# Division/CUDA-RayTracing

Measured on AMD Instinct MI355X. Metric: Mrays/s + achieved HBM GB/s, Stanford bunny 1920x1080x8spp @1/2/4/8 GPU, higher is better.
Workload: dtype f32

## Files before the change

### cuda-raytracing_amd/__init__.py

```python
import contextlib
import ctypes
import os

import numpy as np
import torch

PKG_DIR = os.path.dirname(os.path.abspath(__file__))
ROOT_DIR = os.path.dirname(PKG_DIR)
LIB_PATH = os.path.join(PKG_DIR, "librt_hip.so")
EXP_LIB_PATH = os.path.join(PKG_DIR, "librt_hip_exp.so")
ASSETS_DIR = os.path.join(ROOT_DIR, "assets")

RT_RENDER_STATS = 1
RT_RENDER_VALIDATE = 16
TRACERS = {"fast": 0, "ref": 2, "flat": 4, "wavefront": 8}
STAT_NAMES = ("segments", "nodes", "tri_tests", "tri_accepts", "sphere_accepts", "hits", "misses", "cycles_tree_cut",
              "wave_small_iters", "lane_small", "wave_big_tris", "lane_big_tris", "wave_segment_iters",
              "lane_segments", "tree_nodes", "tree_tri_tests", "cycles_small", "cycles_big", "cycles_total",
              "rounds_coop", "rounds_shared", "coop_rays", "cycles_tree_clusters", "cycles_tree_tris",
              "big_tests", "twin_decided", "twin_tests", "wave_big_iters", "defer_end2", "defer_redo", None, None)
STAT_COUNT = len(STAT_NAMES)
SCENES = {"bunny": 0, "bunny4": 1, "plane1m": 2}

REFERENCE_SPP = 5
# ... 248 lines not shown
    "rt_scene_camera": (None, [_P, ctypes.POINTER(GPUCamera)]),
    "rt_scene_host_arrays": (_SZ, [_P, ctypes.POINTER(_P), ctypes.POINTER(_SZ), ctypes.POINTER(_P),
                                   ctypes.POINTER(_SZ), ctypes.POINTER(_P), ctypes.POINTER(_SZ), ctypes.POINTER(_P)]),
    "rt_scene_bvh_max_depth": (_I, [_P]),
    "rt_scene_materials": (_I, [_P, _P, ctypes.POINTER(_SZ)]),
    "rt_scene_spheres": (_I, [_P, _P, ctypes.POINTER(_SZ)]),
    "rt_bvh_build_device": (_I, [_P, _U32, _P, _U32, _P, _P, ctypes.POINTER(_U32), ctypes.POINTER(_I), _P]),
    "rt_scene_mirror_info": (_I, [_P, ctypes.POINTER(_SZ), ctypes.POINTER(_SZ), ctypes.POINTER(_SZ)]),
    "rt_scene_mirror_copy": (_I, [_P, _P, _P, _P]),
    "rt_scene_mirror_nodes": (_I, [_P, _P, ctypes.POINTER(_SZ)]),
    "rt_scene_mirror_face_leaf": (_I, [_P, _P, ctypes.POINTER(_SZ)]),
    "rt_scene_mirror_twins": (_I, [_P, _P, ctypes.POINTER(_SZ), _P, ctypes.POINTER(_SZ)]),
    "rt_mirror_build_check": (_I, [_P, _SZ, _P, _SZ, _P, _SZ, _P, _SZ, _P, ctypes.POINTER(ctypes.c_int)]),
    "rt_cluster_cull_host": (_I, [_P, _P, ctypes.c_float, _P]),
    "rt_twin_check_host": (_I, [_P, _P, _P]),
    "rt_variant_host": (None, [_P, _P]),
    "rt_family_has_mode_host": (_I, [_I, _I]),
    "rt_xorwow_jump_matrix": (_I, [_I, ctypes.POINTER(ctypes.c_uint32)]),
    "rt_xorwow_init_host": (None, [_U32, _U64, _P]),
}

_lib = None


class RTError(RuntimeError):
    pass


def lib():
    global _lib
# ... 148 lines not shown
        _check(lib().rt_scene_mirror_face_leaf(self.handle, None, ctypes.byref(n)), "rt_scene_mirror_face_leaf")
        out = np.zeros(n.value, dtype=np.uint32)
        if n.value:
            _check(lib().rt_scene_mirror_face_leaf(self.handle, out.ctypes.data, ctypes.byref(n)), "rt_scene_mirror_face_leaf")
        return out

    def mirror_twins(self):
        import numpy as np
        nq, nu = ctypes.c_size_t(), ctypes.c_size_t()
        _check(lib().rt_scene_mirror_twins(self.handle, None, ctypes.byref(nq), None, ctypes.byref(nu)), "rt_scene_mirror_twins")
        q = np.zeros((nq.value, 28), dtype=np.float32)
        u = np.zeros((nu.value, 16), dtype=np.float32)
        _check(lib().rt_scene_mirror_twins(self.handle, q.ctypes.data, ctypes.byref(nq), u.ctypes.data, ctypes.byref(nu)),
               "rt_scene_mirror_twins")
        return q, u

    def materials(self):
        n = ctypes.c_size_t()
        _check(lib().rt_scene_materials(self.handle, None, ctypes.byref(n)), "rt_scene_materials")
        out = np.zeros((n.value, 16), dtype=np.float32)
        if n.value:
            _check(lib().rt_scene_materials(self.handle, out.ctypes.data, ctypes.byref(n)), "rt_scene_materials")
        return out

    def spheres(self):
        n = ctypes.c_size_t()
        _check(lib().rt_scene_spheres(self.handle, None, ctypes.byref(n)), "rt_scene_spheres")
        out = np.zeros((n.value, 8), dtype=np.float32)
        if n.value:
            _check(lib().rt_scene_spheres(self.handle, out.ctypes.data, ctypes.byref(n)), "rt_scene_spheres")
# ... 1033 lines not shown
```

### cuda-raytracing_amd/csrc/host_hooks.hip

```cpp
#include <hip/hip_runtime.h>

#include "rt_abi.h"
#include "rt_device.h"
#include "rt_math.h"
#include "rt_common.h"
#include "leaftree.h"
#include "rt_fast.h"
#include "mirror.h"
#include "rt_render.h"

static_assert(MIRROR_BIG_LEAF == (uint32_t)rtfast::BIG, "pair records exist for exactly the big leaves");

extern "C" int rt_experimental_loaded() { return rtk::experimental_kernels() ? 1 : 0; }

extern "C" int rt_twin_check_host(const float rec[12], const float o[3], const float nd[3]) {
    using rtm::f3;
    const f3 O = rtm::mk(o[0], o[1], o[2]), N = rtm::mk(nd[0], nd[1], nd[2]), v0 = rtm::mk(rec[0], rec[1], rec[2]);
    const f3 e1 = rtm::mk(rec[3], rec[4], rec[5]), e2 = rtm::mk(rec[6], rec[7], rec[8]);
    auto glm = [&](f3 a, f3 b, float* det, float* u, float* v, float* uv) {
        const f3 p = rtm::cross(N, b);
        *det = rtm::dot(a, p);
        const f3 dist = rtm::sub(O, v0);
        *u = rtm::dot(dist, p);
        *v = rtm::dot(N, rtm::cross(dist, a));
        *uv = *u + *v;
    };
    auto ok = [](float det, float u, float v, float uv) {
        const bool neg = signbit(det);
        const float ad = fabsf(det), su = neg ? -u : u, sv = neg ? -v : v, suv = neg ? -uv : uv;
        return ad > 1.1920928955078125e-07f && !(su < 0.0f || su > ad) && !(sv < 0.0f || suv > ad);
    };
    float d, u, v, uv, d2, u2, v2, uv2;
    glm(e1, e2, &d, &u, &v, &uv);
    glm(e2, e1, &d2, &u2, &v2, &uv2);
    const f3 dist = rtm::sub(O, v0);
    const float dn = (fabsf(dist.x) + fabsf(dist.y)) + fabsf(dist.z);
    float kd, ke;
    rt_twin_bounds(rec, &kd, &ke);
    return (rtfast::twin_rejected(d, u, v, uv, dn, kd, ke) ? 1 : 0) | (ok(d2, u2, v2, uv2) ? 2 : 0) | (ok(d, u, v, uv) ? 4 : 0);
}

extern "C" void rt_variant_host(const int32_t in[9], int32_t out[5]) {
    const rtk::VariantInput vi{(uint32_t)in[0], in[1] != 0, in[2] != 0, in[3] != 0, in[4] != 0,
                               in[5] != 0, in[6] != 0, in[7], in[8] != 0};
    const rtk::Variant v = rtk::choose_variant(vi);
    out[0] = v.family, out[1] = v.mode, out[2] = v.stack, out[3] = v.needs_plugin, out[4] = v.use_entry;
}

template <int... MODES>
static bool one_of(int mode) { return ((mode == MODES) || ...); }
extern "C" int rt_family_has_mode_host(int family, int mode) {
    switch (family) {
#define RT_FAMILY_CASE(FAM, NAME, STATS, ...) case rtk::FAM: return one_of<__VA_ARGS__>(mode);
        RT_FAST_FAMILIES(RT_FAMILY_CASE)
// ... 19 lines not shown
```

### cuda-raytracing_amd/csrc/mirror.cpp

```cpp
#include "mirror.h"

#include <cstdlib>
#include <functional>

#include "leaftree.h"

#include <algorithm>
#include <atomic>
#include <cmath>
#include <cstring>
#include <map>
#include <mutex>
#include <stdexcept>
#include <string>

namespace {
void put_flat(float* o, const float* p0, const float* p1, const float* p2, uint32_t face) {
    o[0] = p0[0], o[1] = p0[1], o[2] = p0[2];
    o[3] = p1[0] - p0[0], o[4] = p1[1] - p0[1], o[5] = p1[2] - p0[2];
    o[6] = p2[0] - p0[0], o[7] = p2[1] - p0[1], o[8] = p2[2] - p0[2];
    std::memcpy(&o[9], &face, 4);
    o[10] = o[11] = 0.0f;
}
void put_pair(float* q, const float* a, const float* b) {
// ... 4 lines not shown
    std::memcpy(&q[19], &b[9], 4);
}
}

void rt_twin_bounds(const float* r, float* kd, float* ke) {
    const double U = std::ldexp(1.0, -24);
    const double n1 = std::fabs((double)r[3]) + std::fabs((double)r[4]) + std::fabs((double)r[5]);
    const double n2 = std::fabs((double)r[6]) + std::fabs((double)r[7]) + std::fabs((double)r[8]);
    const double w = 1.0 + std::ldexp(1.0, -20);
    *kd = (float)(10.0001 * U * n1 * n2 * w * w);
    *ke = (float)(10.0001 * U * std::max(n1, n2) * w * w);
}

namespace {
bool build_twins(const float* tris, uint32_t first, uint32_t count, std::vector<float>& quads,
                 std::vector<float>& units, uint32_t* nq, uint32_t* nu) {
    if (count >= 0xffffu) return false;
    auto key = [&](uint32_t i, bool swapped) {
        const float* r = &tris[(size_t)(first + i) * 12];
        std::string k(reinterpret_cast<const char*>(r), 12);
        k.append(reinterpret_cast<const char*>(r + (swapped ? 6 : 3)), 12);
        k.append(reinterpret_cast<const char*>(r + (swapped ? 3 : 6)), 12);
        return k;
    };
    std::map<std::string, std::vector<uint32_t>> by;
    for (uint32_t i = 0; i < count; i++) by[key(i, false)].push_back(i);
    std::vector<char> used(count, 0);
    std::vector<std::pair<uint32_t, uint32_t>> un;
    for (uint32_t i = 0; i < count; i++) {
        if (used[i]) continue;
        used[i] = 1;
// ... 31 lines not shown
        float kd, ke;
        rt_twin_bounds(ra, &kd, &ke);
        q[20] = un[u].second == none ? -1.0f : kd, q[22] = ke;
        rt_twin_bounds(rb, &kd, &ke);
        q[21] = (!hb || un[u + 1].second == none) ? -1.0f : kd, q[23] = ke;
        const uint32_t wa = packed(un[u].first, un[u].second), wb = hb ? packed(un[u + 1].first, un[u + 1].second) : none;
        const uint32_t fa = face(un[u].second), fb = hb ? face(un[u + 1].second) : none;
        std::memcpy(&q[24], &wa, 4);
        std::memcpy(&q[25], &wb, 4);
        std::memcpy(&q[26], &fa, 4);
        std::memcpy(&q[27], &fb, 4);
        quads.insert(quads.end(), q, q + 28);
    }
    *nq = (uint32_t)((un.size() + 1) / 2);
    *nu = (uint32_t)un.size();
    return true;
}
}

void rt_build_mirror(const GPUBVHNode* nodes, size_t node_count, const uint32_t* fi, size_t index_count,
                     const GPUFace* faces, size_t face_count, const GPUVertex* verts, size_t vertex_count,
                     MirrorHost* out) {
    auto bad = [](const char* what) { throw std::runtime_error(std::string("mirror: ") + what); };
    out->tris.assign(index_count * 12, 0.0f);
    for (size_t i = 0; i < index_count; i++) {
        const uint32_t f = fi[i];
        if (f >= face_count) bad("face index out of range");
        const GPUFace& fc = faces[f];
        if (fc.v0 >= vertex_count || fc.v1 >= vertex_count || fc.v2 >= vertex_count) bad("vertex index out of range");
        put_flat(&out->tris[i * 12], verts[fc.v0].position, verts[fc.v1].position, verts[fc.v2].position, f);
// ... 68 lines not shown
        rt_get_build_options(&opt);
        if (nd.prim_count >= opt.leaf_tree_min) {
            LeafTreeParams prm;
            prm.cut_clusters = opt.cut_clusters;
            prm.split_angle = opt.split_angle;
            prm.cluster_max = opt.cluster_max;
            po = rt_build_leaf_tree(&out->tris[(size_t)nd.first_index * 12], nd.prim_count, prm, out->tree, out->ltris);
            rt_build_leaf_flat(out->tree, po, prm, out->flat);
            if (out->ltris.size() / 12 >= (1u << 26)) bad("leaf trees too large (record index >= 2^26)");
            roots.push_back(po);
            pf = 2;
            std::memcpy(&lead[10], &po, 4);
            std::memcpy(&lead[11], &pf, 4);
            continue;
        }
        float scr[20];
        rt_build_options so;
        rt_get_build_options(&so);
        LeafTreeParams sp;
        sp.split_angle = so.split_angle;
        pf = 1;
        if (so.leaf_screens && rt_build_leaf_screen(&out->tris[(size_t)nd.first_index * 12], nd.prim_count, sp, scr)) {
            out->pairs.insert(out->pairs.end(), scr, scr + 20);
            pf = 3;
            out->screens++;
        }
        po = (uint32_t)(out->pairs.size() / 20);
        std::memcpy(&lead[10], &po, 4);
        std::memcpy(&lead[11], &pf, 4);
        for (uint32_t j = 0; j < nd.prim_count; j += 2) {
            float q[20];
            put_pair(q, &out->tris[((size_t)nd.first_index + j) * 12],
                     j + 1 < nd.prim_count ? &out->tris[((size_t)nd.first_index + j + 1) * 12] : nullptr);
            out->pairs.insert(out->pairs.end(), q, q + 20);
        }
        const uint32_t qb = (uint32_t)(out->quads.size() / 28), ub = (uint32_t)(out->units.size() / 16);
        uint32_t nq = 0, nu = 0;
        if (twins_ok && build_twins(out->tris.data(), nd.first_index, nd.prim_count, out->quads, out->units, &nq, &nu)) {
            float* second = &out->tris[((size_t)nd.first_index + 1) * 12];
            float* third = &out->tris[((size_t)nd.first_index + 2) * 12];
            std::memcpy(&second[10], &qb, 4);
            std::memcpy(&second[11], &nq, 4);
            std::memcpy(&third[10], &ub, 4);
            std::memcpy(&third[11], &nu, 4);
        }
    }
    const uint32_t nl = (uint32_t)(out->ltris.size() / 12);
    for (uint32_t r : roots) std::memcpy(&out->tree[(size_t)r * 16 + 12], &nl, 4);
    rt_build_treelets(nodes, node_count, out->treelets);
    rt_build_private_nodes(nodes, node_count, out->nodes);
    out->face_leaf.clear();
    if (!out->pairs.empty() || !out->tree.empty()) {
        std::vector<uint32_t> fl(face_count, FACE_NO_LEAF);
        const size_t nn = out->nodes.size() / 8;
        for (size_t k = 0; k < nn; k++) {
            uint32_t first, count;
            std::memcpy(&first, &out->nodes[k * 8 + 6], 4);
            std::memcpy(&count, &out->nodes[k * 8 + 7], 4);
            if (count == 0 || (size_t)first + count > index_count) continue;
// ... 244 lines not shown
```

### cuda-raytracing_amd/csrc/rt_fast.h

```cpp
#pragma once

#include "rt_variant.h"

namespace rtfast {

constexpr int BIG = 8;
constexpr int WAVE = 64;

using rtm::f3;

struct Ray {
    f3 o, d, nd, r;
    bool fast;
};

__device__ __forceinline__ bool in_range_or_zero(float v, float lo, float hi) {
    const float a = fabsf(v);
    return v == 0.0f || (a >= lo && a <= hi);
}

__device__ __forceinline__ Ray make_ray(f3 o, f3 d, f3 nd, bool scene_fast) {
    Ray R;
    R.o = o, R.d = d, R.nd = nd;
    R.r = rtm::mk(1.0f / d.x, 1.0f / d.y, 1.0f / d.z);
// ... 200 lines not shown
            return true;
        }
    }
    return false;
}

__device__ __forceinline__ bool tri_ok(float det, float u, float v, float uv) {
    const float eps = 1.1920928955078125e-07f;
    const uint32_t sgn = __float_as_uint(det) & 0x80000000u;
    const float adet = fabsf(det);
    const float su = __uint_as_float(__float_as_uint(u) ^ sgn);
    const float sv = __uint_as_float(__float_as_uint(v) ^ sgn);
    const float suv = __uint_as_float(__float_as_uint(uv) ^ sgn);
    return adet > eps && !(su < 0.0f || su > adet) && !(sv < 0.0f || suv > adet);
}

__device__ __forceinline__ bool tri_accept(f3 o, f3 nd, float4 A, float4 B, float4 Cc, float best, float* t_o,
                                           float* bx, float* by, bool* nan) {
    const f3 e1 = rtm::mk(A.w, B.x, B.y), e2 = rtm::mk(B.z, B.w, Cc.x);
    const f3 p = rtm::cross(nd, e2);
    const float det = rtm::dot(e1, p);
    const f3 dist = rtm::sub(o, rtm::mk(A.x, A.y, A.z));
    const float u = rtm::dot(dist, p);
    const f3 perp = rtm::cross(dist, e1);
    const float v = rtm::dot(nd, perp);
    const float uv = u + v;
    if (!tri_ok(det, u, v, uv)) return false;
    const float inv_det = 1.0f / det;
    const float t = rtm::dot(e2, perp) * inv_det;
    *nan = *nan || (t != t);
// ... 21 lines not shown
}
__device__ __forceinline__ Pair ld_pair_scalar(ConstF4 base, uint32_t p) {
    return make_pair(base[5 * p], base[5 * p + 1], base[5 * p + 2], base[5 * p + 3], base[5 * p + 4]);
}
__device__ __forceinline__ Pair ld_pair(const float4* base, uint32_t p) {
#if defined(RT_ADDR64)
    const f4v* q = reinterpret_cast<const f4v*>(base) + 5 * (size_t)p;
#else
    const f4v* q = reinterpret_cast<const f4v*>(reinterpret_cast<const char*>(base) + p * 80u);
#endif
    return make_pair(q[0], q[1], q[2], q[3], q[4]);
}

struct PairEval {
    f2 det, u, v, uv, qx, qy, qz;
    f2 dn;
};
__device__ __forceinline__ PairEval pair_eval(f3 o, f3 nd, const Pair& P) {
    const f2 ndx = nd.x, ndy = nd.y, ndz = nd.z;
    const f2 px = ndy * P.e2z - P.e2y * ndz;
    const f2 py = ndz * P.e2x - P.e2z * ndx;
    const f2 pz = ndx * P.e2y - P.e2x * ndy;
    PairEval E;
    E.det = (P.e1x * px + P.e1y * py) + P.e1z * pz;
    const f2 dx = o.x - P.v0x, dy = o.y - P.v0y, dz = o.z - P.v0z;
    E.u = (dx * px + dy * py) + dz * pz;
    E.qx = dy * P.e1z - P.e1y * dz;
    E.qy = dz * P.e1x - P.e1z * dx;
    E.qz = dx * P.e1y - P.e1x * dy;
    E.v = (ndx * E.qx + ndy * E.qy) + ndz * E.qz;
    E.uv = E.u + E.v;
    E.dn = f2{(fabsf(dx.x) + fabsf(dy.x)) + fabsf(dz.x), (fabsf(dx.y) + fabsf(dy.y)) + fabsf(dz.y)};
    return E;
}

__device__ __forceinline__ float pair_t(const Pair& P, const PairEval& E, int k, float* inv) {
    const float det = k ? E.det.y : E.det.x;
    *inv = 1.0f / det;
    const f3 e2 = k ? rtm::mk(P.e2x.y, P.e2y.y, P.e2z.y) : rtm::mk(P.e2x.x, P.e2y.x, P.e2z.x);
    const f3 q = k ? rtm::mk(E.qx.y, E.qy.y, E.qz.y) : rtm::mk(E.qx.x, E.qy.x, E.qz.x);
    return rtm::dot(e2, q) * *inv;
}

__device__ __forceinline__ void pair_test(const Ray& R, const Pair& P, Hit& h) {
    const PairEval E = pair_eval(R.o, R.nd, P);
    const bool oka = tri_ok(E.det.x, E.u.x, E.v.x, E.uv.x);
    const bool okb = tri_ok(E.det.y, E.u.y, E.v.y, E.uv.y);
// ... 1 lines not shown
        float inv;
        const float t = pair_t(P, E, 0, &inv);
        if (!(t >= h.best || t < 0.0f)) h.best = t, h.kind = 2, h.id = P.fa, h.bx = E.u.x * inv, h.by = E.v.x * inv;
    }
    if (okb) {
        float inv;
        const float t = pair_t(P, E, 1, &inv);
        if (!(t >= h.best || t < 0.0f)) h.best = t, h.kind = 2, h.id = P.fb, h.bx = E.u.y * inv, h.by = E.v.y * inv;
    }
}

extern "C" __device__ uint32_t __ockl_wfred_min_u32(uint32_t);

constexpr uint32_t NO_POS = 0xffffffffu;

RT_HD bool twin_rejected(float det, float u, float v, float uv, float dn, float kd, float ke) {
    const bool neg = signbit(det);
    const float ad = fabsf(det);
    const float su = neg ? -u : u, sv = neg ? -v : v, suv = neg ? -uv : uv;
    if (!(ad + fabsf(su) + fabsf(sv) + dn < 0x1p100f)) return false;
    const float m = ke * dn + 0x1p-90f;
    const float kdd = kd + 0x1p-90f;
    const float top = (ad + kdd) * (1.0f + 0x1p-20f);
    if (top <= 1.1920928955078125e-07f) return true;
    if (!(ad > kdd * (1.0f + 0x1p-20f))) return false;
    if (sv < -m || su < -m) return true;
    if (sv > (ad + kdd + m) * (1.0f + 0x1p-20f)) return true;
    return suv * (1.0f - 0x1p-20f) > (ad + kdd + 2.001f * m) * (1.0f + 0x1p-20f);
}

__device__ __forceinline__ void offer(float t, uint32_t pos, uint32_t id, float bx, float by, Hit& h, uint32_t& bpos,
                                      bool& nan) {
    if (t != t) {
        nan = true;
        return;
    }
    const bool take = (t >= 0.0f) & ((t < h.best) | ((t == h.best) & (bpos != NO_POS) & (pos < bpos)));
    if (take) h.best = t, h.kind = 2, h.id = id, h.bx = bx, h.by = by, bpos = pos;
}

__device__ __forceinline__ void tri_offer(f3 o, f3 nd, f3 v0, f3 e1, f3 e2, uint32_t pos, uint32_t face, Hit& h,
                                          uint32_t& bpos, bool& nan) {
    const f3 p = rtm::cross(nd, e2);
    const float det = rtm::dot(e1, p);
    const f3 dist = rtm::sub(o, v0);
    const float u = rtm::dot(dist, p);
    const f3 perp = rtm::cross(dist, e1);
    const float v = rtm::dot(nd, perp);
    if (tri_ok(det, u, v, u + v)) {
        const float inv_det = 1.0f / det;
        offer(rtm::dot(e2, perp) * inv_det, pos, face, u * inv_det, v * inv_det, h, bpos, nan);
    }
}

template <bool TIMING, class C>
__device__ __forceinline__ void quad_test(f3 o, f3 nd, const Pair& P, f4v bnd, ConstF4 q6, Hit& h, uint32_t& bpos,
                                          bool& nan, C& c) {
    const PairEval E = pair_eval(o, nd, P);
    const bool oka = tri_ok(E.det.x, E.u.x, E.v.x, E.uv.x), okb = tri_ok(E.det.y, E.u.y, E.v.y, E.uv.y);
    const bool twa = bnd.x >= 0.0f && !twin_rejected(E.det.x, E.u.x, E.v.x, E.uv.x, E.dn.x, bnd.x, bnd.z);
    const bool twb = bnd.y >= 0.0f && !twin_rejected(E.det.y, E.u.y, E.v.y, E.uv.y, E.dn.y, bnd.y, bnd.w);
    if (TIMING) {
        c.big_tests += 2;
        c.tw_test += (uint32_t)twa + (uint32_t)twb;
        c.tw_dec += (uint32_t)(bnd.x >= 0.0f && !twa) + (uint32_t)(bnd.y >= 0.0f && !twb);
    }
    if (oka || okb || twa || twb) {
        const f4v W = *q6;
        const uint32_t wa = __float_as_uint(W.x), wb = __float_as_uint(W.y);
        if (oka) {
            float inv;
            const float t = pair_t(P, E, 0, &inv);
            offer(t, wa & 0xffffu, P.fa, E.u.x * inv, E.v.x * inv, h, bpos, nan);
        }
        if (okb) {
            float inv;
            const float t = pair_t(P, E, 1, &inv);
            offer(t, wb & 0xffffu, P.fb, E.u.y * inv, E.v.y * inv, h, bpos, nan);
        }
        if (twa)
            tri_offer(o, nd, rtm::mk(P.v0x.x, P.v0y.x, P.v0z.x), rtm::mk(P.e2x.x, P.e2y.x, P.e2z.x),
                      rtm::mk(P.e1x.x, P.e1y.x, P.e1z.x), wa >> 16, __float_as_uint(W.z), h, bpos, nan);
        if (twb)
            tri_offer(o, nd, rtm::mk(P.v0x.y, P.v0y.y, P.v0z.y), rtm::mk(P.e2x.y, P.e2y.y, P.e2z.y),
                      rtm::mk(P.e1x.y, P.e1y.y, P.e1z.y), wb >> 16, __float_as_uint(W.w), h, bpos, nan);
    }
}

template <bool TIMING, class C>
__device__ __forceinline__ void unit_test(f3 o, f3 nd, float4 A, float4 B, float4 Cc, float4 D, Hit& h, uint32_t& bpos,
                                          bool& nan, C& c) {
    const f3 v0 = rtm::mk(A.x, A.y, A.z), e1 = rtm::mk(A.w, B.x, B.y), e2 = rtm::mk(B.z, B.w, Cc.x);
    const f3 p = rtm::cross(nd, e2);
    const float det = rtm::dot(e1, p);
    const f3 dist = rtm::sub(o, v0);
    const float u = rtm::dot(dist, p);
    const f3 perp = rtm::cross(dist, e1);
    const float v = rtm::dot(nd, perp);
    const float uv = u + v;
    const uint32_t w = __float_as_uint(Cc.w);
    if (tri_ok(det, u, v, uv)) {
        const float inv_det = 1.0f / det;
        offer(rtm::dot(e2, perp) * inv_det, w & 0xffffu, __float_as_uint(Cc.y), u * inv_det, v * inv_det, h, bpos, nan);
    }
    const float dn = (fabsf(dist.x) + fabsf(dist.y)) + fabsf(dist.z);
    const bool tw = D.x >= 0.0f && !twin_rejected(det, u, v, uv, dn, D.x, D.y);
    if (TIMING) c.big_tests++, c.tw_test += (uint32_t)tw, c.tw_dec += (uint32_t)(D.x >= 0.0f && !tw);
    if (tw) tri_offer(o, nd, v0, e2, e1, w >> 16, __float_as_uint(Cc.z), h, bpos, nan);
}

__device__ __forceinline__ void leaf_sequential(const float4* tris, uint32_t f0, uint32_t c0, f3 o, f3 nd, Hit& h) {
    for (uint32_t j = 0; j < c0; j++) {
        const float4 A = tris[3 * (f0 + j)], B = tris[3 * (f0 + j) + 1], Cc = tris[3 * (f0 + j) + 2];
        float t, x, y;
        bool dummy = false;
        if (tri_accept(o, nd, A, B, Cc, h.best, &t, &x, &y, &dummy)) {
            h.best = t, h.kind = 2, h.bx = x, h.by = y;
            h.id = __float_as_uint(Cc.y);
        }
    }
}

// ... 47 lines not shown
            continue;
        }
        const bool has = bi != 0xffffffffu;
        const uint32_t mk = __ockl_wfred_min_u32(has ? tkey(bt) : 0xffffffffu);
        const uint32_t mi = __ockl_wfred_min_u32(has && tkey(bt) == mk ? bi : 0xffffffffu);
        if (mi != 0xffffffffu) {
            const int wl = (int)((mi >> 1) & 63u);
            const float wbx = bcast(bx, wl), wby = bcast(by, wl), wt = bcast(bt, wl);
            const uint32_t wid = (uint32_t)__builtin_amdgcn_readlane((int)bid, wl);
            if ((int)lane == r) h.best = wt, h.kind = 2, h.bx = wbx, h.by = wby, h.id = wid;
        }
    }
}

template <bool TIMING, class C>
__device__ __forceinline__ void coop_units(const float4* tris, const float4* un, uint32_t nu, unsigned long long big,
                                           uint32_t f0, uint32_t c0, const Ray& R, Hit& h, C& c) {
    const uint32_t lane = threadIdx.x & 63u;
    unsigned long long m = big;
    while (m) {
        const int r = __ffsll((long long)m) - 1;
        m &= m - 1;
        const f3 rox = rtm::mk(bcast(R.o.x, r), bcast(R.o.y, r), bcast(R.o.z, r));
        const f3 nd = rtm::mk(bcast(R.nd.x, r), bcast(R.nd.y, r), bcast(R.nd.z, r));
        Hit L;
        L.best = bcast(h.best, r), L.kind = 0, L.id = 0, L.bx = L.by = 0.0f;
        uint32_t bpos = NO_POS;
        bool nan = !(L.best == L.best);
        for (uint32_t q = lane; q < nu; q += 64u)
            unit_test<TIMING>(rox, nd, un[4 * q], un[4 * q + 1], un[4 * q + 2], un[4 * q + 3], L, bpos, nan, c);
        if (TIMING && lane == 0) c.big_iters += (nu + 63u) / 64u;
        if (__ballot(nan)) {
            if ((int)lane == r) leaf_sequential(tris, f0, c0, R.o, R.nd, h);
            continue;
        }
        const bool has = bpos != NO_POS;
        const uint32_t mk = __ockl_wfred_min_u32(has ? tkey(L.best) : 0xffffffffu);
        const uint32_t mi = __ockl_wfred_min_u32(has && tkey(L.best) == mk ? bpos : 0xffffffffu);
        if (mi != 0xffffffffu) {
            const int wl = __ffsll((long long)__ballot(has && bpos == mi)) - 1;
            const float wt = bcast(L.best, wl), wbx = bcast(L.bx, wl), wby = bcast(L.by, wl);
            const uint32_t wid = (uint32_t)__builtin_amdgcn_readlane((int)L.id, wl);
            if ((int)lane == r) h.best = wt, h.kind = 2, h.bx = wbx, h.by = wby, h.id = wid;
        }
    }
// ... 481 lines not shown
            return at_tree;
        }
    }
    const int l0 = __ffsll((long long)big) - 1;
    const uint32_t f0 = __builtin_amdgcn_readlane(T.first, l0);
    const uint32_t c0 = __builtin_amdgcn_readlane(T.count, l0);
    if (STATS) {
        uint32_t mx = waiting ? T.count : 0u;
        for (int off = 32; off > 0; off >>= 1) mx = max(mx, (uint32_t)__shfl_xor((int)mx, off));
        c.w_big += (threadIdx.x & 63) == 0 ? mx : 0;
        c.l_big += waiting ? T.count : 0;
    }
    if (__ballot(waiting && T.first == f0) == big) {
        const f4v lead = ((ConstF4)(tris + 3 * (size_t)f0))[2];
        const uint32_t k = (uint32_t)__popcll(big);
        if (!STATS && (MODE & BIG_MASK) < BIG_SCALAR && (LEAN || quads) && (__float_as_uint(lead.w) & 1u)) {
            const f4v l2 = ((ConstF4)(tris + 3 * (size_t)f0 + 3))[2];
            const f4v l3 = ((ConstF4)(tris + 3 * (size_t)f0 + 6))[2];
            const uint32_t nq = __float_as_uint(l2.w), nu = __float_as_uint(l3.w);
            const uint32_t cw = (tune >> 21) & 7u;
            if (nu && (tune & 1u) == 0 && k * (70u * ((nu + 63u) / 64u) + 70u) * (cw ? cw : 4u) < 4u * 95u * nq) {
                coop_units<(MODE & TIMING_BIT) != 0>(tris, units + 4 * (size_t)__float_as_uint(l3.z), nu, big, f0, c0, R, h, c);
                if (MODE & TIMING_BIT) c.r_coop++, c.coop_rays += k;
                return waiting;
            }
            if (nq) {
                if (MODE & TIMING_BIT) c.r_shared++;
                const Hit h0 = h;
                uint32_t bpos = NO_POS;
                bool nan = !(h.best == h.best);
                ConstF4 qs = (ConstF4)(quads + 7 * (size_t)__float_as_uint(l2.z));
                for (uint32_t q = 0; q < nq; q++, qs += 7) {
                    const Pair P = make_pair(qs[0], qs[1], qs[2], qs[3], qs[4]);
                    const f4v bnd = qs[5];
                    if (waiting) quad_test<(MODE & TIMING_BIT) != 0>(R.o, R.nd, P, bnd, qs + 6, h, bpos, nan, c);
                }
                if (MODE & TIMING_BIT) c.big_iters += nq;
                if (waiting && nan) {
                    h = h0;
                    leaf_sequential(tris, f0, c0, R.o, R.nd, h);
                }
                return waiting;
            }
        }
        if (!STATS && (MODE & BIG_MASK) < BIG_SCALAR && (LEAN || pairs) && (__float_as_uint(lead.w) & 1u)) {
            const float4* lp = pairs + 5 * (size_t)__float_as_uint(lead.z);
            const uint32_t np = (c0 + 1u) / 2u, chunks = (np + 63u) / 64u;
            const uint32_t cchunks = (c0 + 63u) / 64u;
            if ((MODE & BIG_MASK) == BIG_PAIRS && (tune & 1u) == 0 && k * (40u * chunks + 60u) < 40u * np) {
                coop_leaf(tris, lp, big, f0, c0, R, h);
// ... 373 lines not shown
```

### cuda-raytracing_amd/csrc/scene.cpp

```cpp
#include "scene.h"
#include "mirror.h"

#include <algorithm>
#include <cmath>
#include <array>
#include <cstdio>
#include <cstring>
#include <fstream>

namespace RayTracing {

using rtm::add;
using rtm::cross;
using rtm::divs;
using rtm::mk;
using rtm::muls;
using rtm::normalize;
using rtm::sub;

DeviceMemory::DeviceMemory(size_t n) : size(n) {
    if (rt_malloc(&memory, n == 0 ? 16 : n) != 0) throw std::runtime_error("allocation failed");
}
DeviceMemory::~DeviceMemory() {
    if (memory) rt_free(memory);
// ... 639 lines not shown
    MirrorHost m;
    if (host_mirror(s, &m) != 0) return -1;
    *count = m.nodes.size() / 8;
    if (nodes) std::memcpy(nodes, m.nodes.data(), m.nodes.size() * 4);
    return 0;
}
int rt_scene_mirror_twins(rt_scene* s, float* quads, size_t* quad_count, float* units, size_t* unit_count) {
    MirrorHost m;
    if (host_mirror(s, &m) != 0) return -1;
    *quad_count = m.quads.size() / 28;
    *unit_count = m.units.size() / 16;
    if (quads) std::memcpy(quads, m.quads.data(), m.quads.size() * 4);
    if (units) std::memcpy(units, m.units.data(), m.units.size() * 4);
    return 0;
}
int rt_scene_mirror_face_leaf(rt_scene* s, uint32_t* leaf, size_t* count) {
    MirrorHost m;
    if (host_mirror(s, &m) != 0) return -1;
    *count = m.face_leaf.size();
    if (leaf) std::memcpy(leaf, m.face_leaf.data(), m.face_leaf.size() * 4);
    return 0;
}
int rt_scene_materials(rt_scene* s, void* out, size_t* count) {
    if (!s || !count) {
        rt_internal_set_error("rt_scene_materials: null argument");
        return -1;
    }
    const std::vector<GPUMaterial> gm = s->scene.HostMaterials();
    *count = gm.size();
    if (out) {
// ... 61 lines not shown
```

### include/rt_abi.h

```cpp
#ifndef RT_ABI_H
#define RT_ABI_H

#include <stddef.h>
#include <stdint.h>

#ifdef __cplusplus
extern "C" {
#endif

#if defined(__cplusplus)
#define RT_ALIGNAS(n) alignas(n)
#else
#define RT_ALIGNAS(n) _Alignas(n)
#endif


typedef struct GPUCamera {
    float origin[3];
    float viewport_worldspace_size[2];
    float aspect;
    float horizontal[3];
    float vertical[3];
    float lower_left_corner[3];
} GPUCamera;
// ... 607 lines not shown
    int32_t entry_frontier;
} rt_build_options;
void rt_get_build_options(rt_build_options* out);
int rt_set_build_options(const rt_build_options* options);

uint64_t rt_entry_table_builds(void);

int rt_bvh_build_device(const GPUVertex* vertices, uint32_t vertex_count, const GPUFace* faces, uint32_t face_count,
                        GPUBVHNode* nodes_out, uint32_t* face_indices_out, uint32_t* node_count_out,
                        int* max_depth_out, void* stream);

int rt_scene_mirror_info(rt_scene* scene, size_t* tri_records, size_t* tree_nodes, size_t* tree_tri_records);
int rt_scene_mirror_copy(rt_scene* scene, float* tris, float* tree, float* tree_tris);
int rt_cluster_cull_host(const float origin[3], const float nd[3], float best, const float node[16]);
int rt_twin_check_host(const float rec[12], const float origin[3], const float nd[3]);
void rt_variant_host(const int32_t in[9], int32_t out[5]);
int rt_family_has_mode_host(int family, int mode);
int rt_scene_mirror_nodes(rt_scene* scene, GPUBVHNode* nodes, size_t* count);
int rt_scene_mirror_twins(rt_scene* scene, float* quads, size_t* quad_count, float* units, size_t* unit_count);
int rt_scene_mirror_face_leaf(rt_scene* scene, uint32_t* leaf, size_t* count);

int rt_mirror_build_check(const GPUBVHNode* nodes, size_t node_count, const uint32_t* face_indices, size_t index_count,
                          const GPUFace* faces, size_t face_count, const GPUVertex* vertices, size_t vertex_count,
                          uint32_t* meta, int* twins);

int rt_xorwow_jump_matrix(int k, uint32_t out[800]);
void rt_xorwow_init_host(uint32_t seed, uint64_t subsequence, rt_rng_state* out);

#ifdef __cplusplus
}
#endif

#endif
```

Measured before the change: 2375.

## Hoist twin-rejection bounds to per-leaf and per-ray-visit constants in big-leaf tests

```diff
diff --git a/cuda-raytracing_amd/__init__.py b/cuda-raytracing_amd/__init__.py
--- a/cuda-raytracing_amd/__init__.py
+++ b/cuda-raytracing_amd/__init__.py
@@ -286,6 +286,9 @@
     "rt_mirror_build_check": (_I, [_P, _SZ, _P, _SZ, _P, _SZ, _P, _SZ, _P, ctypes.POINTER(ctypes.c_int)]),
     "rt_cluster_cull_host": (_I, [_P, _P, ctypes.c_float, _P]),
     "rt_twin_check_host": (_I, [_P, _P, _P]),
+    "rt_twin_check_bounds_host": (_I, [_P, _P, _P, _P]),
+    "rt_twin_visit_host": (None, [_P, _P, _P, ctypes.c_float, _P]),
+    "rt_scene_mirror_leaf_twin": (_I, [_P, _U32, _P]),
     "rt_variant_host": (None, [_P, _P]),
     "rt_family_has_mode_host": (_I, [_I, _I]),
     "rt_xorwow_jump_matrix": (_I, [_I, ctypes.POINTER(ctypes.c_uint32)]),
@@ -464,6 +467,12 @@
         _check(lib().rt_scene_mirror_twins(self.handle, q.ctypes.data, ctypes.byref(nq), u.ctypes.data, ctypes.byref(nu)),
                "rt_scene_mirror_twins")
         return q, u
+
+    def mirror_leaf_twin(self, first):
+        import numpy as np
+        rec = np.zeros(12, dtype=np.float32)
+        _check(lib().rt_scene_mirror_leaf_twin(self.handle, int(first), rec.ctypes.data), "rt_scene_mirror_leaf_twin")
+        return rec
 
     def materials(self):
         n = ctypes.c_size_t()
diff --git a/cuda-raytracing_amd/csrc/host_hooks.hip b/cuda-raytracing_amd/csrc/host_hooks.hip
--- a/cuda-raytracing_amd/csrc/host_hooks.hip
+++ b/cuda-raytracing_amd/csrc/host_hooks.hip
@@ -13,8 +13,9 @@
 
 extern "C" int rt_experimental_loaded() { return rtk::experimental_kernels() ? 1 : 0; }
 
-extern "C" int rt_twin_check_host(const float rec[12], const float o[3], const float nd[3]) {
+static int twin_check(const float rec[12], const float o[3], const float nd[3], const float* bounds) {
     using rtm::f3;
+    using namespace rtfast;
     const f3 O = rtm::mk(o[0], o[1], o[2]), N = rtm::mk(nd[0], nd[1], nd[2]), v0 = rtm::mk(rec[0], rec[1], rec[2]);
     const f3 e1 = rtm::mk(rec[3], rec[4], rec[5]), e2 = rtm::mk(rec[6], rec[7], rec[8]);
     auto glm = [&](f3 a, f3 b, float* det, float* u, float* v, float* uv) {
@@ -33,11 +34,40 @@
     float d, u, v, uv, d2, u2, v2, uv2;
     glm(e1, e2, &d, &u, &v, &uv);
     glm(e2, e1, &d2, &u2, &v2, &uv2);
-    const f3 dist = rtm::sub(O, v0);
-    const float dn = (fabsf(dist.x) + fabsf(dist.y)) + fabsf(dist.z);
-    float kd, ke;
-    rt_twin_bounds(rec, &kd, &ke);
-    return (rtfast::twin_rejected(d, u, v, uv, dn, kd, ke) ? 1 : 0) | (ok(d2, u2, v2, uv2) ? 2 : 0) | (ok(d, u, v, uv) ? 4 : 0);
+    const int glm_bits = (ok(d2, u2, v2, uv2) ? 2 : 0) | (ok(d, u, v, uv) ? 4 : 0);
+    if (!bounds) {
+        const f3 dist = rtm::sub(O, v0);
+        const float dn = (fabsf(dist.x) + fabsf(dist.y)) + fabsf(dist.z);
+        float kd, ke;
+        rt_twin_bounds(rec, &kd, &ke);
+        return (twin_rejected(d, u, v, uv, dn, kd, ke) ? 1 : 0) | glm_bits;
+    }
+    const float dn = bounds[2], m = bounds[1] * dn + 0x1p-90f, m2 = 2.001f * m;
+    const float kdd = bounds[0] + 0x1p-90f, kdd1 = kdd * (1.0f + 0x1p-20f);
+    const bool scalar = twin_rejected_pre(d, u, v, uv, dn, m, m2, kdd, kdd1);
+    bool same = true;
+    for (int half = 0; half < 2; half++) {
+        auto two = [&](float x) { return half ? f2{0.0f, x} : f2{x, 0.0f}; };
+        const f2 D = two(d);
+        const TwinFold<f2> F = twin_fold<f2>(D, two(u), two(v), two(uv), f2{copysignf(1.0f, D.x), copysignf(1.0f, D.y)});
+        const TwinLimits<f2> L = twin_limits<f2>(F.ad, F.suv, m, m2, kdd);
+        const bool packed = half ? twin_decide(F.ad.y, F.su.y, F.sv.y, dn, m, kdd1, L.top.y, L.lim_v.y, L.lim_uv.y, L.suv_lo.y)
+                                 : twin_decide(F.ad.x, F.su.x, F.sv.x, dn, m, kdd1, L.top.x, L.lim_v.x, L.lim_uv.x, L.suv_lo.x);
+        same = same && packed == scalar;
+        const bool okp = half ? tri_ok_folded(F.ad.y, F.su.y, F.sv.y, F.suv.y) : tri_ok_folded(F.ad.x, F.su.x, F.sv.x, F.suv.x);
+        same = same && okp == ok(d, u, v, uv);
+    }
+    return (scalar ? 1 : 0) | glm_bits | (same ? 0 : 8);
+}
+extern "C" int rt_twin_check_host(const float rec[12], const float o[3], const float nd[3]) {
+    return twin_check(rec, o, nd, nullptr);
+}
+extern "C" int rt_twin_check_bounds_host(const float rec[12], const float o[3], const float nd[3], const float bounds[3]) {
+    return twin_check(rec, o, nd, bounds);
+}
+extern "C" void rt_twin_visit_host(const float o[3], const float lo[3], const float hi[3], float ke, float out[3]) {
+    const rtfast::TwinVisit V = rtfast::twin_visit(rtm::mk(o[0], o[1], o[2]), rtm::mk(lo[0], lo[1], lo[2]), rtm::mk(hi[0], hi[1], hi[2]), ke);
+    out[0] = V.dn, out[1] = V.m, out[2] = V.m2;
 }
 
 extern "C" void rt_variant_host(const int32_t in[9], int32_t out[5]) {
diff --git a/cuda-raytracing_amd/csrc/mirror.cpp b/cuda-raytracing_amd/csrc/mirror.cpp
--- a/cuda-raytracing_amd/csrc/mirror.cpp
+++ b/cuda-raytracing_amd/csrc/mirror.cpp
@@ -42,7 +42,7 @@
 
 namespace {
 bool build_twins(const float* tris, uint32_t first, uint32_t count, std::vector<float>& quads,
-                 std::vector<float>& units, uint32_t* nq, uint32_t* nu) {
+                 std::vector<float>& units, uint32_t* nq, uint32_t* nu, float leaf[20]) {
     if (count >= 0xffffu) return false;
     auto key = [&](uint32_t i, bool swapped) {
         const float* r = &tris[(size_t)(first + i) * 12];
@@ -104,6 +104,27 @@
     }
     *nq = (uint32_t)((un.size() + 1) / 2);
     *nu = (uint32_t)un.size();
+    float KD = 0.0f, KE = 0.0f, lo[3], hi[3];
+    for (size_t u = 0; u < un.size(); u++) {
+        const float* r = &tris[(size_t)(first + un[u].first) * 12];
+        for (int k = 0; k < 3; k++) {
+            lo[k] = u ? std::min(lo[k], r[k]) : r[k];
+            hi[k] = u ? std::max(hi[k], r[k]) : r[k];
+        }
+        if (un[u].second == none) continue;
+        float kd, ke;
+        rt_twin_bounds(r, &kd, &ke);
+        KD = std::max(KD, kd), KE = std::max(KE, ke);
+    }
+    auto up = [](double x) {
+        const float f = (float)x;
+        return (double)f < x ? std::nextafter(f, INFINITY) : f;
+    };
+    std::fill(leaf, leaf + 20, 0.0f);
+    leaf[0] = KD, leaf[1] = KE;
+    leaf[2] = up((double)KD + std::ldexp(1.0, -90));
+    leaf[3] = up((double)leaf[2] * (1.0 + std::ldexp(1.0, -20)));
+    for (int k = 0; k < 3; k++) leaf[4 + k] = lo[k], leaf[8 + k] = hi[k];
     return true;
 }
 }
@@ -202,6 +223,18 @@
             std::memcpy(&lead[11], &pf, 4);
             continue;
         }
+        const uint32_t qb = (uint32_t)(out->quads.size() / 28), ub = (uint32_t)(out->units.size() / 16);
+        uint32_t nq = 0, nu = 0;
+        float twin_rec[20];
+        if (twins_ok && build_twins(out->tris.data(), nd.first_index, nd.prim_count, out->quads, out->units, &nq, &nu, twin_rec)) {
+            float* second = &out->tris[((size_t)nd.first_index + 1) * 12];
+            float* third = &out->tris[((size_t)nd.first_index + 2) * 12];
+            std::memcpy(&second[10], &qb, 4);
+            std::memcpy(&second[11], &nq, 4);
+            std::memcpy(&third[10], &ub, 4);
+            std::memcpy(&third[11], &nu, 4);
+            out->pairs.insert(out->pairs.end(), twin_rec, twin_rec + 20);
+        }
         float scr[20];
         rt_build_options so;
         rt_get_build_options(&so);
@@ -221,16 +254,6 @@
             put_pair(q, &out->tris[((size_t)nd.first_index + j) * 12],
                      j + 1 < nd.prim_count ? &out->tris[((size_t)nd.first_index + j + 1) * 12] : nullptr);
             out->pairs.insert(out->pairs.end(), q, q + 20);
-        }
-        const uint32_t qb = (uint32_t)(out->quads.size() / 28), ub = (uint32_t)(out->units.size() / 16);
-        uint32_t nq = 0, nu = 0;
-        if (twins_ok && build_twins(out->tris.data(), nd.first_index, nd.prim_count, out->quads, out->units, &nq, &nu)) {
-            float* second = &out->tris[((size_t)nd.first_index + 1) * 12];
-            float* third = &out->tris[((size_t)nd.first_index + 2) * 12];
-            std::memcpy(&second[10], &qb, 4);
-            std::memcpy(&second[11], &nq, 4);
-            std::memcpy(&third[10], &ub, 4);
-            std::memcpy(&third[11], &nu, 4);
         }
     }
     const uint32_t nl = (uint32_t)(out->ltris.size() / 12);
diff --git a/cuda-raytracing_amd/csrc/rt_fast.h b/cuda-raytracing_amd/csrc/rt_fast.h
--- a/cuda-raytracing_amd/csrc/rt_fast.h
+++ b/cuda-raytracing_amd/csrc/rt_fast.h
@@ -238,6 +238,9 @@
     const float suv = __uint_as_float(__float_as_uint(uv) ^ sgn);
     return adet > eps && !(su < 0.0f || su > adet) && !(sv < 0.0f || suv > adet);
 }
+RT_HD bool tri_ok_folded(float adet, float su, float sv, float suv) {
+    return adet > 1.1920928955078125e-07f && !(su < 0.0f || su > adet) && !(sv < 0.0f || suv > adet);
+}
 
 __device__ __forceinline__ bool tri_accept(f3 o, f3 nd, float4 A, float4 B, float4 Cc, float best, float* t_o,
                                            float* bx, float* by, bool* nan) {
@@ -289,7 +292,6 @@
 
 struct PairEval {
     f2 det, u, v, uv, qx, qy, qz;
-    f2 dn;
 };
 __device__ __forceinline__ PairEval pair_eval(f3 o, f3 nd, const Pair& P) {
     const f2 ndx = nd.x, ndy = nd.y, ndz = nd.z;
@@ -305,7 +307,6 @@
     E.qz = dx * P.e1y - P.e1x * dy;
     E.v = (ndx * E.qx + ndy * E.qy) + ndz * E.qz;
     E.uv = E.u + E.v;
-    E.dn = f2{(fabsf(dx.x) + fabsf(dy.x)) + fabsf(dz.x), (fabsf(dx.y) + fabsf(dy.y)) + fabsf(dz.y)};
     return E;
 }
 
@@ -337,19 +338,68 @@
 
 constexpr uint32_t NO_POS = 0xffffffffu;
 
+template <class V>
+struct TwinFold {
+    V ad, su, sv, suv;
+};
+template <class V>
+RT_HD TwinFold<V> twin_fold(V det, V u, V v, V uv, V s) {
+    return TwinFold<V>{det * s, u * s, v * s, uv * s};
+}
+template <class V>
+struct TwinLimits {
+    V top, lim_v, lim_uv, suv_lo;
+};
+RT_HD float add_each(float a, float b) { return a + b; }
+RT_HD f2 add_each(f2 a, float b) { return f2{a.x + b, a.y + b}; }
+template <class V>
+RT_HD TwinLimits<V> twin_limits(V ad, V suv, float m, float m2, V kdd) {
+    const V up = 1.0f + 0x1p-20f, down = 1.0f - 0x1p-20f;
+    const V t0 = ad + kdd;
+    return TwinLimits<V>{t0 * up, add_each(t0, m) * up, add_each(t0, m2) * up, suv * down};
+}
+RT_HD bool twin_decide(float ad, float su, float sv, float guard_dn, float m, float kdd1, float top, float lim_v,
+                       float lim_uv, float suv_lo) {
+    const bool in_range = ad + fabsf(su) + fabsf(sv) + guard_dn < 0x1p100f;
+    const bool out = (sv < -m) | (su < -m) | (sv > lim_v) | (suv_lo > lim_uv);
+    return in_range & ((top <= 1.1920928955078125e-07f) | ((ad > kdd1) & out));
+}
+RT_HD bool twin_rejected_pre(float det, float u, float v, float uv, float guard_dn, float m, float m2, float kdd,
+                             float kdd1) {
+    const TwinFold<float> F = twin_fold<float>(det, u, v, uv, copysignf(1.0f, det));
+    const TwinLimits<float> L = twin_limits<float>(F.ad, F.suv, m, m2, kdd);
+    return twin_decide(F.ad, F.su, F.sv, guard_dn, m, kdd1, L.top, L.lim_v, L.lim_uv, L.suv_lo);
+}
 RT_HD bool twin_rejected(float det, float u, float v, float uv, float dn, float kd, float ke) {
-    const bool neg = signbit(det);
-    const float ad = fabsf(det);
-    const float su = neg ? -u : u, sv = neg ? -v : v, suv = neg ? -uv : uv;
-    if (!(ad + fabsf(su) + fabsf(sv) + dn < 0x1p100f)) return false;
     const float m = ke * dn + 0x1p-90f;
     const float kdd = kd + 0x1p-90f;
-    const float top = (ad + kdd) * (1.0f + 0x1p-20f);
-    if (top <= 1.1920928955078125e-07f) return true;
-    if (!(ad > kdd * (1.0f + 0x1p-20f))) return false;
-    if (sv < -m || su < -m) return true;
-    if (sv > (ad + kdd + m) * (1.0f + 0x1p-20f)) return true;
-    return suv * (1.0f - 0x1p-20f) > (ad + kdd + 2.001f * m) * (1.0f + 0x1p-20f);
+    return twin_rejected_pre(det, u, v, uv, dn, m, 2.001f * m, kdd, kdd * (1.0f + 0x1p-20f));
+}
+
+struct TwinVisit {
+    float dn, m, m2;
+};
+RT_HD float twin_visit_dn(f3 o, f3 lo, f3 hi) {
+    const float ax = fmaxf(fabsf(o.x - lo.x), fabsf(o.x - hi.x));
+    const float ay = fmaxf(fabsf(o.y - lo.y), fabsf(o.y - hi.y));
+    const float az = fmaxf(fabsf(o.z - lo.z), fabsf(o.z - hi.z));
+    return ((ax + ay) + az) * (1.0f + 0x1p-20f);
+}
+RT_HD TwinVisit twin_visit_from(float dn, float ke) {
+    TwinVisit V;
+    V.dn = dn;
+    V.m = ke * dn + 0x1p-90f;
+    V.m2 = 2.001f * V.m;
+    return V;
+}
+RT_HD TwinVisit twin_visit(f3 o, f3 lo, f3 hi, float ke) { return twin_visit_from(twin_visit_dn(o, lo, hi), ke); }
+struct TwinLeaf {
+    float ke, kdd, kdd1;
+    f3 lo, hi;
+};
+__device__ __forceinline__ TwinLeaf ld_twin_leaf(ConstF4 rec) {
+    const f4v k = rec[0], lo = rec[1], hi = rec[2];
+    return TwinLeaf{k.y, k.z, k.w, rtm::mk(lo.x, lo.y, lo.z), rtm::mk(hi.x, hi.y, hi.z)};
 }
 
 __device__ __forceinline__ void offer(float t, uint32_t pos, uint32_t id, float bx, float by, Hit& h, uint32_t& bpos,
@@ -377,12 +427,15 @@
 }
 
 template <bool TIMING, class C>
-__device__ __forceinline__ void quad_test(f3 o, f3 nd, const Pair& P, f4v bnd, ConstF4 q6, Hit& h, uint32_t& bpos,
-                                          bool& nan, C& c) {
+__device__ __forceinline__ void quad_test(f3 o, f3 nd, const Pair& P, f4v bnd, const TwinLeaf& K, const TwinVisit& B,
+                                          ConstF4 q6, Hit& h, uint32_t& bpos, bool& nan, C& c) {
     const PairEval E = pair_eval(o, nd, P);
-    const bool oka = tri_ok(E.det.x, E.u.x, E.v.x, E.uv.x), okb = tri_ok(E.det.y, E.u.y, E.v.y, E.uv.y);
-    const bool twa = bnd.x >= 0.0f && !twin_rejected(E.det.x, E.u.x, E.v.x, E.uv.x, E.dn.x, bnd.x, bnd.z);
-    const bool twb = bnd.y >= 0.0f && !twin_rejected(E.det.y, E.u.y, E.v.y, E.uv.y, E.dn.y, bnd.y, bnd.w);
+    const f2 s = f2{copysignf(1.0f, E.det.x), copysignf(1.0f, E.det.y)};
+    const TwinFold<f2> F = twin_fold<f2>(E.det, E.u, E.v, E.uv, s);
+    const bool oka = tri_ok_folded(F.ad.x, F.su.x, F.sv.x, F.suv.x), okb = tri_ok_folded(F.ad.y, F.su.y, F.sv.y, F.suv.y);
+    const TwinLimits<f2> L = twin_limits<f2>(F.ad, F.suv, B.m, B.m2, K.kdd);
+    const bool twa = (bnd.x >= 0.0f) & !twin_decide(F.ad.x, F.su.x, F.sv.x, B.dn, B.m, K.kdd1, L.top.x, L.lim_v.x, L.lim_uv.x, L.suv_lo.x);
+    const bool twb = (bnd.y >= 0.0f) & !twin_decide(F.ad.y, F.su.y, F.sv.y, B.dn, B.m, K.kdd1, L.top.y, L.lim_v.y, L.lim_uv.y, L.suv_lo.y);
     if (TIMING) {
         c.big_tests += 2;
         c.tw_test += (uint32_t)twa + (uint32_t)twb;
@@ -391,16 +444,12 @@
     if (oka || okb || twa || twb) {
         const f4v W = *q6;
         const uint32_t wa = __float_as_uint(W.x), wb = __float_as_uint(W.y);
-        if (oka) {
-            float inv;
-            const float t = pair_t(P, E, 0, &inv);
-            offer(t, wa & 0xffffu, P.fa, E.u.x * inv, E.v.x * inv, h, bpos, nan);
-        }
-        if (okb) {
-            float inv;
-            const float t = pair_t(P, E, 1, &inv);
-            offer(t, wb & 0xffffu, P.fb, E.u.y * inv, E.v.y * inv, h, bpos, nan);
-        }
+        if (oka)
+            tri_offer(o, nd, rtm::mk(P.v0x.x, P.v0y.x, P.v0z.x), rtm::mk(P.e1x.x, P.e1y.x, P.e1z.x),
+                      rtm::mk(P.e2x.x, P.e2y.x, P.e2z.x), wa & 0xffffu, P.fa, h, bpos, nan);
+        if (okb)
+            tri_offer(o, nd, rtm::mk(P.v0x.y, P.v0y.y, P.v0z.y), rtm::mk(P.e1x.y, P.e1y.y, P.e1z.y),
+                      rtm::mk(P.e2x.y, P.e2y.y, P.e2z.y), wb & 0xffffu, P.fb, h, bpos, nan);
         if (twa)
             tri_offer(o, nd, rtm::mk(P.v0x.x, P.v0y.x, P.v0z.x), rtm::mk(P.e2x.x, P.e2y.x, P.e2z.x),
                       rtm::mk(P.e1x.x, P.e1y.x, P.e1z.x), wa >> 16, __float_as_uint(W.z), h, bpos, nan);
@@ -411,8 +460,8 @@
 }
 
 template <bool TIMING, class C>
-__device__ __forceinline__ void unit_test(f3 o, f3 nd, float4 A, float4 B, float4 Cc, float4 D, Hit& h, uint32_t& bpos,
-                                          bool& nan, C& c) {
+__device__ __forceinline__ void unit_test(f3 o, f3 nd, float4 A, float4 B, float4 Cc, float kd, const TwinLeaf& K,
+                                          Hit& h, uint32_t& bpos, bool& nan, C& c) {
     const f3 v0 = rtm::mk(A.x, A.y, A.z), e1 = rtm::mk(A.w, B.x, B.y), e2 = rtm::mk(B.z, B.w, Cc.x);
     const f3 p = rtm::cross(nd, e2);
     const float det = rtm::dot(e1, p);
@@ -427,8 +476,9 @@
         offer(rtm::dot(e2, perp) * inv_det, w & 0xffffu, __float_as_uint(Cc.y), u * inv_det, v * inv_det, h, bpos, nan);
     }
     const float dn = (fabsf(dist.x) + fabsf(dist.y)) + fabsf(dist.z);
-    const bool tw = D.x >= 0.0f && !twin_rejected(det, u, v, uv, dn, D.x, D.y);
-    if (TIMING) c.big_tests++, c.tw_test += (uint32_t)tw, c.tw_dec += (uint32_t)(D.x >= 0.0f && !tw);
+    const TwinVisit V = twin_visit_from(dn, K.ke);
+    const bool tw = (kd >= 0.0f) & !twin_rejected_pre(det, u, v, uv, V.dn, V.m, V.m2, K.kdd, K.kdd1);
+    if (TIMING) c.big_tests++, c.tw_test += (uint32_t)tw, c.tw_dec += (uint32_t)(kd >= 0.0f && !tw);
     if (tw) tri_offer(o, nd, v0, e2, e1, w >> 16, __float_as_uint(Cc.z), h, bpos, nan);
 }
 
@@ -506,8 +556,8 @@
 }
 
 template <bool TIMING, class C>
-__device__ __forceinline__ void coop_units(const float4* tris, const float4* un, uint32_t nu, unsigned long long big,
-                                           uint32_t f0, uint32_t c0, const Ray& R, Hit& h, C& c) {
+__device__ __forceinline__ void coop_units(const float4* tris, const float4* un, uint32_t nu, const TwinLeaf& K,
+                                           unsigned long long big, uint32_t f0, uint32_t c0, const Ray& R, Hit& h, C& c) {
     const uint32_t lane = threadIdx.x & 63u;
     unsigned long long m = big;
     while (m) {
@@ -520,7 +570,7 @@
         uint32_t bpos = NO_POS;
         bool nan = !(L.best == L.best);
         for (uint32_t q = lane; q < nu; q += 64u)
-            unit_test<TIMING>(rox, nd, un[4 * q], un[4 * q + 1], un[4 * q + 2], un[4 * q + 3], L, bpos, nan, c);
+            unit_test<TIMING>(rox, nd, un[4 * q], un[4 * q + 1], un[4 * q + 2], un[4 * q + 3].x, K, L, bpos, nan, c);
         if (TIMING && lane == 0) c.big_iters += (nu + 63u) / 64u;
         if (__ballot(nan)) {
             if ((int)lane == r) leaf_sequential(tris, f0, c0, R.o, R.nd, h);
@@ -1032,13 +1082,15 @@
     if (__ballot(waiting && T.first == f0) == big) {
         const f4v lead = ((ConstF4)(tris + 3 * (size_t)f0))[2];
         const uint32_t k = (uint32_t)__popcll(big);
-        if (!STATS && (MODE & BIG_MASK) < BIG_SCALAR && (LEAN || quads) && (__float_as_uint(lead.w) & 1u)) {
+        if (!STATS && (MODE & BIG_MASK) < BIG_SCALAR && (LEAN || (quads && pairs)) && (__float_as_uint(lead.w) & 1u)) {
             const f4v l2 = ((ConstF4)(tris + 3 * (size_t)f0 + 3))[2];
             const f4v l3 = ((ConstF4)(tris + 3 * (size_t)f0 + 6))[2];
             const uint32_t nq = __float_as_uint(l2.w), nu = __float_as_uint(l3.w);
+            const uint32_t pk = __float_as_uint(lead.w);
+            const TwinLeaf K = ld_twin_leaf((ConstF4)(pairs + 5 * (size_t)(__float_as_uint(lead.z) - 1u - ((pk >> 1) & 1u))));
             const uint32_t cw = (tune >> 21) & 7u;
             if (nu && (tune & 1u) == 0 && k * (70u * ((nu + 63u) / 64u) + 70u) * (cw ? cw : 4u) < 4u * 95u * nq) {
-                coop_units<(MODE & TIMING_BIT) != 0>(tris, units + 4 * (size_t)__float_as_uint(l3.z), nu, big, f0, c0, R, h, c);
+                coop_units<(MODE & TIMING_BIT) != 0>(tris, units + 4 * (size_t)__float_as_uint(l3.z), nu, K, big, f0, c0, R, h, c);
                 if (MODE & TIMING_BIT) c.r_coop++, c.coop_rays += k;
                 return waiting;
             }
@@ -1047,11 +1099,12 @@
                 const Hit h0 = h;
                 uint32_t bpos = NO_POS;
                 bool nan = !(h.best == h.best);
+                const TwinVisit B = twin_visit(R.o, K.lo, K.hi, K.ke);
                 ConstF4 qs = (ConstF4)(quads + 7 * (size_t)__float_as_uint(l2.z));
                 for (uint32_t q = 0; q < nq; q++, qs += 7) {
                     const Pair P = make_pair(qs[0], qs[1], qs[2], qs[3], qs[4]);
                     const f4v bnd = qs[5];
-                    if (waiting) quad_test<(MODE & TIMING_BIT) != 0>(R.o, R.nd, P, bnd, qs + 6, h, bpos, nan, c);
+                    if (waiting) quad_test<(MODE & TIMING_BIT) != 0>(R.o, R.nd, P, bnd, K, B, qs + 6, h, bpos, nan, c);
                 }
                 if (MODE & TIMING_BIT) c.big_iters += nq;
                 if (waiting && nan) {
diff --git a/cuda-raytracing_amd/csrc/scene.cpp b/cuda-raytracing_amd/csrc/scene.cpp
--- a/cuda-raytracing_amd/csrc/scene.cpp
+++ b/cuda-raytracing_amd/csrc/scene.cpp
@@ -677,6 +677,23 @@
     if (units) std::memcpy(units, m.units.data(), m.units.size() * 4);
     return 0;
 }
+int rt_scene_mirror_leaf_twin(rt_scene* s, uint32_t first, float rec[12]) {
+    MirrorHost m;
+    if (host_mirror(s, &m) != 0) return -1;
+    uint32_t po = 0, pf = 0, nq = 0;
+    if ((size_t)first + 2 < m.tris.size() / 12) {
+        std::memcpy(&po, &m.tris[(size_t)first * 12 + 10], 4);
+        std::memcpy(&pf, &m.tris[(size_t)first * 12 + 11], 4);
+        std::memcpy(&nq, &m.tris[((size_t)first + 1) * 12 + 11], 4);
+    }
+    const uint32_t back = 1u + (pf == 3u ? 1u : 0u);
+    if (!m.twins || (pf != 1u && pf != 3u) || nq == 0 || po < back || (size_t)po * 20 > m.pairs.size()) {
+        rt_internal_set_error("rt_scene_mirror_leaf_twin: not the first record of a big leaf with twin records");
+        return -1;
+    }
+    std::memcpy(rec, &m.pairs[(size_t)(po - back) * 20], 12 * 4);
+    return 0;
+}
 int rt_scene_mirror_face_leaf(rt_scene* s, uint32_t* leaf, size_t* count) {
     MirrorHost m;
     if (host_mirror(s, &m) != 0) return -1;
diff --git a/include/rt_abi.h b/include/rt_abi.h
--- a/include/rt_abi.h
+++ b/include/rt_abi.h
@@ -645,10 +645,13 @@
 int rt_scene_mirror_copy(rt_scene* scene, float* tris, float* tree, float* tree_tris);
 int rt_cluster_cull_host(const float origin[3], const float nd[3], float best, const float node[16]);
 int rt_twin_check_host(const float rec[12], const float origin[3], const float nd[3]);
+int rt_twin_check_bounds_host(const float rec[12], const float origin[3], const float nd[3], const float bounds[3]);
+void rt_twin_visit_host(const float origin[3], const float lo[3], const float hi[3], float ke, float out[3]);
 void rt_variant_host(const int32_t in[9], int32_t out[5]);
 int rt_family_has_mode_host(int family, int mode);
 int rt_scene_mirror_nodes(rt_scene* scene, GPUBVHNode* nodes, size_t* count);
 int rt_scene_mirror_twins(rt_scene* scene, float* quads, size_t* quad_count, float* units, size_t* unit_count);
+int rt_scene_mirror_leaf_twin(rt_scene* scene, uint32_t first, float rec[12]);
 int rt_scene_mirror_face_leaf(rt_scene* scene, uint32_t* leaf, size_t* count);
 
 int rt_mirror_build_check(const GPUBVHNode* nodes, size_t node_count, const uint32_t* face_indices, size_t index_count,
```

New measurement: 2429 (median of 6 runs). 1.02x the previous value.
